# XiaoWang-Github/ORBIT-2

Hardware: AMD Instinct MI355X
Metric: climate-grid samples/sec/node (fwd+bwd), interm_1b ERA5 1.4°→0.25°, 1/2/4/8 GPUs (higher is better)
Workload: dtype bf16

## Files before the change

orbit-2_amd/csrc/common.h:

```cpp
#pragma once
#include <hip/hip_runtime.h>
#include <stdint.h>
#include <type_traits>

#define O2_OK 0
#define O2_ERR_ARG (-1)
#define O2_ERR_LAUNCH (-2)
#define O2_ERR_UNSUPPORTED (-3)

typedef unsigned short bf16_t;
typedef __attribute__((ext_vector_type(8))) short bf16x8;
typedef __attribute__((ext_vector_type(4))) short bf16x4;
typedef __attribute__((ext_vector_type(4))) float f32x4;
typedef __attribute__((ext_vector_type(16))) float f32x16;
typedef __attribute__((ext_vector_type(4))) unsigned int u32x4;
typedef __attribute__((ext_vector_type(2))) unsigned int u32x2;

#define LDS_PTR(T, p) ((__attribute__((address_space(3))) T*)(p))
#define GLB_PTR(T, p) ((const __attribute__((address_space(1))) T*)(p))

__device__ __forceinline__ float bf2f(bf16_t u) { return __uint_as_float(((unsigned)u) << 16); }
__device__ __forceinline__ bf16_t f2bf(float f) { return __builtin_bit_cast(unsigned short, (__bf16)f); }
typedef __attribute__((ext_vector_type(2))) float o2_f32x2;
typedef __attribute__((ext_vector_type(2))) __bf16 o2_bf16x2;
__device__ __forceinline__ unsigned pack_bf2(float lo, float hi) {
  const o2_f32x2 v = {lo, hi};
  return __builtin_bit_cast(unsigned, __builtin_convertvector(v, o2_bf16x2));
}
__device__ __forceinline__ void unpack8(const u32x4 r, float* f) {
#pragma unroll
  for (int k = 0; k < 4; ++k) { f[2 * k] = bf2f((bf16_t)(r[k] & 0xffff)); f[2 * k + 1] = bf2f((bf16_t)(r[k] >> 16)); }
}
__device__ __forceinline__ u32x4 pack8(const float* v) {
  u32x4 o;
#pragma unroll
  for (int k = 0; k < 4; ++k) o[k] = pack_bf2(v[2 * k], v[2 * k + 1]);
  return o;
}

__device__ __forceinline__ void glds16(const void* gsrc, void* lds_wave_base) {
  __builtin_amdgcn_global_load_lds(GLB_PTR(void, gsrc), LDS_PTR(void, lds_wave_base), 16, 0, 0);
}
__device__ __forceinline__ void glds4(const void* gsrc, void* lds_wave_base) {
  __builtin_amdgcn_global_load_lds(GLB_PTR(void, gsrc), LDS_PTR(void, lds_wave_base), 4, 0, 0);
}
__device__ __forceinline__ void glds16_asm(const void* gbase_uniform, uint32_t lane_byte_off, uint32_t lds_dst_uniform) {
  unsigned keep;
  asm volatile("s_mov_b32 %0, m0\n\ts_mov_b32 m0, %3\n\ts_nop 0\n\tglobal_load_lds_dwordx4 %1, %2\n\ts_mov_b32 m0, %0"
               : "=&s"(keep)
               : "v"(lane_byte_off), "s"(gbase_uniform), "s"(lds_dst_uniform)
               : "memory");
}
__device__ __forceinline__ void glds4_asm(const void* gbase_uniform, uint32_t lane_byte_off, uint32_t lds_dst_uniform) {
  unsigned keep;
  asm volatile("s_mov_b32 %0, m0\n\ts_mov_b32 m0, %3\n\ts_nop 0\n\tglobal_load_lds_dword %1, %2\n\ts_mov_b32 m0, %0"
               : "=&s"(keep)
               : "v"(lane_byte_off), "s"(gbase_uniform), "s"(lds_dst_uniform)
               : "memory");
}
__device__ __forceinline__ bf16x4 lds_tr4(const void* lds_addr) {
  return __builtin_amdgcn_ds_read_tr16_b64_v4i16(LDS_PTR(bf16x4, lds_addr));
}

static __device__ uint64_t o2_seed_salt = 0;
#define O2_DEFINE_SALT_OP(tag)                                                                           \
  namespace {                                                                                            \
  __global__ void o2_salt_kernel_##tag(uint64_t v, int add) { o2_seed_salt = add ? o2_seed_salt + v : v; } \
  }                                                                                                      \
  void o2_salt_op_##tag(uint64_t v, int add, hipStream_t s) {                                            \
    hipLaunchKernelGGL(o2_salt_kernel_##tag, dim3(1), dim3(1), 0, s, v, add);                            \
  }
void o2_salt_op_gemm(uint64_t v, int add, hipStream_t s);
void o2_salt_op_attn(uint64_t v, int add, hipStream_t s);
void o2_salt_op_elem(uint64_t v, int add, hipStream_t s);

__device__ __host__ __forceinline__ uint32_t o2_hash(uint32_t seed_lo, uint32_t seed_hi, uint32_t idx_lo,
                                                      uint32_t idx_hi) {
  const uint32_t t = idx_hi ^ seed_hi;
  uint32_t h = idx_lo ^ seed_lo ^ ((t << 16) | (t >> 16)) ^ (t + (t << 3));
  h ^= h >> 16;
  h *= 0x7FEB352Du;
  h ^= h >> 15;
  h *= 0x846CA68Bu;
  h ^= h >> 16;
  return h;
}
__device__ __forceinline__ uint32_t o2_hash64(uint64_t seed, uint64_t idx) {
  return o2_hash((uint32_t)seed, (uint32_t)(seed >> 32), (uint32_t)idx, (uint32_t)(idx >> 32));
}
__device__ __forceinline__ void o2_drop8(float* f, uint64_t salted_seed, int64_t idx, unsigned thr, float dscale) {
  const uint32_t h0 = o2_hash64(salted_seed, (uint64_t)idx >> 2), h1 = o2_hash64(salted_seed, ((uint64_t)idx >> 2) + 1);
#pragma unroll
  for (int j = 0; j < 4; ++j) {
    f[j] = (((h0 >> (8 * j)) & 0xffu) >= thr) ? f[j] * dscale : 0.f;
    f[4 + j] = (((h1 >> (8 * j)) & 0xffu) >= thr) ? f[4 + j] * dscale : 0.f;
  }
}

#define O2_ATTN_KEY_SALT 0x85EBCA6B9E3779B9ull
__device__ __forceinline__ uint32_t o2_attn_rowhash(uint64_t seed, uint64_t row) { return o2_hash64(seed, row); }
__device__ __forceinline__ uint32_t o2_attn_keyhash(uint64_t seed, uint32_t kg) {
  return o2_hash64(seed ^ O2_ATTN_KEY_SALT, (uint64_t)kg);
}
__device__ __forceinline__ uint32_t o2_attn_mix(uint32_t r, uint32_t k) {
  uint32_t x = (r ^ k) * 0x9E3779B1u;
  return x ^ (x >> 16);
}

__device__ __forceinline__ float gelu_f(float x) { return 0.5f * x * (1.0f + erff(x * 0.70710678118654752f)); }
__device__ __forceinline__ float dgelu_f(float x) {
  const float cdf = 0.5f * (1.0f + erff(x * 0.70710678118654752f));
  const float pdf = 0.3989422804014327f * __expf(-0.5f * x * x);
  return cdf + x * pdf;
}

__device__ __forceinline__ float o2_half_erfc_abs(float x, float& e) {
  const float u = fabsf(x) * 0.70710678118654752f;
  const float t = __builtin_amdgcn_rcpf(fmaf(0.3275911f, u, 1.0f));
  float p = fmaf(1.061405429f, t, -1.453152027f);
  p = fmaf(p, t, 1.421413741f);
  p = fmaf(p, t, -0.284496736f);
  p = fmaf(p, t, 0.254829592f);
  e = __builtin_amdgcn_exp2f(x * x * -0.72134752044448170f);
  return 0.5f * p * t * e;
}
__device__ __forceinline__ float gelu_fast(float x) {
  float e;
  const float y = o2_half_erfc_abs(x, e);
  return x * (x > 0.f ? 1.0f - y : y);
}
__device__ __forceinline__ void gelu_both(float x, float& g, float& dg) {
  float e;
  const float y = o2_half_erfc_abs(x, e);
  const float cdf = x > 0.f ? 1.0f - y : y;
  g = x * cdf;
  dg = cdf + x * 0.3989422804014327f * e;
}
__device__ __forceinline__ float dgelu_fast(float x) {
  float e;
  const float y = o2_half_erfc_abs(x, e);
  return (x > 0.f ? 1.0f - y : y) + x * 0.3989422804014327f * e;
}

__device__ __forceinline__ unsigned pack_q14(float lo, float hi) {
  constexpr float MAGIC = 12582912.0f;
  const float a = __builtin_amdgcn_fmed3f(fmaf(lo, 16384.f, MAGIC), MAGIC - 32768.f, MAGIC + 32767.f);
  const float b = __builtin_amdgcn_fmed3f(fmaf(hi, 16384.f, MAGIC), MAGIC - 32768.f, MAGIC + 32767.f);
  return __builtin_amdgcn_perm(__float_as_uint(b), __float_as_uint(a), 0x05040100u);
}
__device__ __forceinline__ void unpack_q14(unsigned w, float& lo, float& hi) {
  lo = (float)(int)(short)(w & 0xffffu) * (1.0f / 16384.f);
  hi = (float)((int)w >> 16) * (1.0f / 16384.f);
}

__device__ __forceinline__ float wave_sum(float v) {
#pragma unroll
  for (int o = 32; o > 0; o >>= 1) v += __shfl_xor(v, o);
  return v;
}
__device__ __forceinline__ float wave_max(float v) {
#pragma unroll
  for (int o = 32; o > 0; o >>= 1) v = fmaxf(v, __shfl_xor(v, o));
  return v;
}
__device__ __forceinline__ float wave_min(float v) {
#pragma unroll
  for (int o = 32; o > 0; o >>= 1) v = fminf(v, __shfl_xor(v, o));
  return v;
}
__device__ __forceinline__ int wave_sum_i(int v) {
#pragma unroll
  for (int o = 32; o > 0; o >>= 1) v += __shfl_xor(v, o);
  return v;
}
__device__ __forceinline__ int64_t wave_sum_i64(int64_t v) {
#pragma unroll
  for (int o = 32; o > 0; o >>= 1) v += (int64_t)__shfl_xor((long long)v, o);
  return v;
}

template <int TPE>
static __global__ __launch_bounds__(256) void o2_sum_parts_kernel(const float* __restrict__ parts, int nparts, int64_t stride,
                                                                  float* __restrict__ out, int64_t nelem, float scale,
                                                                  int accumulate) {
  const int64_t e = ((int64_t)blockIdx.x * 256 + threadIdx.x) / TPE;
  const int j = threadIdx.x % TPE;
  float s = 0.f;
  if (e < nelem)
    for (int k = j; k < nparts; k += TPE) s += parts[(size_t)k * stride + e];
  if (TPE > 1) {
#pragma unroll
    for (int o = TPE / 2; o > 0; o >>= 1) s += __shfl_xor(s, o);
  }
  if (e < nelem && j == 0) out[e] = accumulate ? out[e] + s * scale : s * scale;
}
static inline void o2_sum_parts(const float* parts, int nparts, int64_t stride, float* out, int64_t nelem, float scale,
                                int accumulate, hipStream_t s) {
  if (nparts > 64) {
    hipLaunchKernelGGL(o2_sum_parts_kernel<32>, dim3((unsigned)((nelem * 32 + 255) / 256)), dim3(256), 0, s, parts, nparts,
                       stride, out, nelem, scale, accumulate);
  } else {
    hipLaunchKernelGGL(o2_sum_parts_kernel<1>, dim3((unsigned)((nelem + 255) / 256)), dim3(256), 0, s, parts, nparts, stride,
                       out, nelem, scale, accumulate);
  }
}

template <int V> using o2_int = std::integral_constant<int, V>;
template <class F> static inline void o2_with_flags(F&& f) { f(); }
template <class F, class... Rest> static inline void o2_with_flags(F&& f, bool flag, Rest... rest) {
  if (flag) o2_with_flags([&](auto... c) { f(std::true_type{}, c...); }, rest...);
  else o2_with_flags([&](auto... c) { f(std::false_type{}, c...); }, rest...);
}

static inline int grid_for(int64_t work_items, int per_block, int max_blocks = 4096) {
  int64_t g = (work_items + per_block - 1) / per_block;
  if (g < 1) g = 1;
  if (g > max_blocks) g = max_blocks;
  return (int)g;
}

#define O2_CHECK_LAUNCH()                                   \
  do {                                                      \
    hipError_t e__ = hipGetLastError();                     \
    if (e__ != hipSuccess) return O2_ERR_LAUNCH;            \
  } while (0)
```

orbit-2_amd/csrc/image.hip:

```cpp
#include "score_sums.h"
#include "../../include/orbit2_hip.h"

namespace {

inline int img_grid(int64_t n) { return grid_for(n, 256, 8192); }

template <bool BWD, bool T_FP32 = false>
__global__ __launch_bounds__(256) void unpatchify_kernel(bf16_t* __restrict__ t, float* __restrict__ img, int B, int C,
                                                         int Hh, int Wh, int p) {
  const int64_t per = (int64_t)C * Hh * Wh;
  const int64_t n = (int64_t)B * per;
  const int wf = Wh / p;
  for (int64_t e = (int64_t)blockIdx.x * 256 + threadIdx.x; e < n; e += (int64_t)gridDim.x * 256) {
    const int b = (int)(e / per);
    int64_t r = e - (int64_t)b * per;
    if (!BWD) {
      const int c = (int)(r / ((int64_t)Hh * Wh));
      r -= (int64_t)c * Hh * Wh;
      const int y = (int)(r / Wh), x = (int)(r - (int64_t)y * Wh);
      const int hh = y / p, pp = y - hh * p, ww = x / p, qq = x - ww * p;
      const int64_t ti = ((((int64_t)hh * wf + ww) * p + pp) * p + qq) * C + c;
      img[e] = T_FP32 ? reinterpret_cast<const float*>(t)[(int64_t)b * per + ti] : bf2f(t[(int64_t)b * per + ti]);
    } else {
      const int c = (int)(r % C);
      int64_t q = r / C;
      const int qq = (int)(q % p); q /= p;
      const int pp = (int)(q % p); q /= p;
      const int ww = (int)(q % wf);
      const int hh = (int)(q / wf);
      t[e] = f2bf(img[(int64_t)b * per + ((int64_t)c * Hh + (hh * p + pp)) * Wh + (ww * p + qq)]);
    }
  }
}

constexpr int CONV_MAXCIN = 8;
constexpr int COB = 16;
__global__ __launch_bounds__(256) void conv3x3_fwd_kernel(const float* __restrict__ in, const int* __restrict__ cidx,
                                                          int in_ctotal, const float* __restrict__ wgt,
                                                          const float* __restrict__ bias, float* __restrict__ out,
                                                          float* __restrict__ pre, const float* __restrict__ addend,
                                                          int Ha, int Wa, int B, int Cin, int Cout, int H, int W,
                                                          int mode, int r) {
  __shared__ float sw[COB * CONV_MAXCIN * 9 + COB];
  const int co0 = blockIdx.y * COB;
  const int nco = (Cout - co0) < COB ? (Cout - co0) : COB;
  for (int e = threadIdx.x; e < nco * Cin * 9; e += 256) sw[e] = wgt[(size_t)co0 * Cin * 9 + e];
  for (int e = threadIdx.x; e < nco; e += 256) sw[COB * CONV_MAXCIN * 9 + e] = bias[co0 + e];
  __syncthreads();
  const int64_t npix = (int64_t)B * H * W;
  for (int64_t px = (int64_t)blockIdx.x * 256 + threadIdx.x; px < npix; px += (int64_t)gridDim.x * 256) {
    const int b = (int)(px / ((int64_t)H * W));
    const int rem = (int)(px - (int64_t)b * H * W);
    const int y = rem / W, x = rem - y * W;
    float nb[CONV_MAXCIN][9];
#pragma unroll
    for (int ci = 0; ci < CONV_MAXCIN; ++ci) {
      if (ci < Cin) {
        const int cs = cidx ? cidx[ci] : ci;
        const float* pl = in + ((size_t)b * in_ctotal + cs) * H * W;
#pragma unroll
        for (int k = 0; k < 9; ++k) {
          const int yy = y + k / 3 - 1, xx = x + k % 3 - 1;
          nb[ci][k] = (yy >= 0 && yy < H && xx >= 0 && xx < W) ? pl[(size_t)yy * W + xx] : 0.f;
        }
      }
    }
    for (int co = 0; co < nco; ++co) {
      float acc = sw[COB * CONV_MAXCIN * 9 + co];
#pragma unroll
      for (int ci = 0; ci < CONV_MAXCIN; ++ci) {
        if (ci < Cin) {
#pragma unroll
          for (int k = 0; k < 9; ++k) acc = fmaf(sw[(co * Cin + ci) * 9 + k], nb[ci][k], acc);
        }
      }
      const int cg = co0 + co;
      if (mode == 0) {
        if (addend) acc += addend[(((size_t)b * Cout + cg) * Ha + y) * Wa + x];
        out[(((size_t)b * Cout + cg) * H + y) * W + x] = acc;
      } else {
        pre[(((size_t)b * Cout + cg) * H + y) * W + x] = acc;
        const int rr = r * r;
        const int oc = cg / rr, sub = cg - oc * rr;
        out[(((size_t)b * (Cout / rr) + oc) * (H * r) + (y * r + sub / r)) * (size_t)(W * r) + (x * r + sub % r)] =
            gelu_f(acc);
      }
    }
  }
}

__device__ __forceinline__ float conv_dpre(const float* __restrict__ dout, const float* __restrict__ pre, int b,
                                           int co, int y, int x, int Cout, int H, int W, int mode, int r) {
  if (mode == 0) return dout[(((size_t)b * Cout + co) * H + y) * W + x];
  const int rr = r * r;
  const int oc = co / rr, sub = co - oc * rr;
  const float d =
      dout[(((size_t)b * (Cout / rr) + oc) * (H * r) + (y * r + sub / r)) * (size_t)(W * r) + (x * r + sub % r)];
  return d * dgelu_f(pre[(((size_t)b * Cout + co) * H + y) * W + x]);
}

__global__ __launch_bounds__(256) void conv3x3_bwd_data_kernel(const float* __restrict__ dout,
                                                               const float* __restrict__ pre,
                                                               const float* __restrict__ wgt, float* __restrict__ din,
                                                               int B, int Cin, int Cout, int H, int W, int mode,
                                                               int r) {
  const int64_t n = (int64_t)B * Cin * H * W;
  for (int64_t e = (int64_t)blockIdx.x * 256 + threadIdx.x; e < n; e += (int64_t)gridDim.x * 256) {
    int64_t q = e;
    const int x = (int)(q % W); q /= W;
    const int y = (int)(q % H); q /= H;
    const int ci = (int)(q % Cin);
    const int b = (int)(q / Cin);
    float acc = 0.f;
    for (int co = 0; co < Cout; ++co) {
#pragma unroll
      for (int k = 0; k < 9; ++k) {
        const int yy = y + 1 - k / 3, xx = x + 1 - k % 3;
        if (yy >= 0 && yy < H && xx >= 0 && xx < W)
          acc = fmaf(conv_dpre(dout, pre, b, co, yy, xx, Cout, H, W, mode, r), wgt[((size_t)co * Cin + ci) * 9 + k],
                     acc);
      }
    }
    din[e] = acc;
  }
}

constexpr int TW = 16, TH = 16;
__global__ __launch_bounds__(256) void conv3x3_bwd_weight_kernel(const float* __restrict__ dout,
                                                                 const float* __restrict__ pre,
                                                                 const float* __restrict__ in,
                                                                 const int* __restrict__ cidx, int in_ctotal,
                                                                 float* __restrict__ ws,
                                                                 int B, int Cin, int Cout, int H, int W, int mode,
                                                                 int r) {
  float* dw = ws + ((size_t)blockIdx.y * gridDim.x + blockIdx.x) * ((size_t)Cout * Cin * 9 + Cout);
  float* dbias = dw + (size_t)Cout * Cin * 9;
  __shared__ float sd[COB][TH][TW];
  __shared__ float si[CONV_MAXCIN][TH + 2][TW + 2];
  const int tiles_x = (W + TW - 1) / TW;
  const int ty0 = (blockIdx.x / tiles_x) * TH, tx0 = (blockIdx.x % tiles_x) * TW;
  const int b = blockIdx.y;
  for (int e = threadIdx.x; e < Cin * (TH + 2) * (TW + 2); e += 256) {
    const int ci = e / ((TH + 2) * (TW + 2));
    const int rem = e - ci * (TH + 2) * (TW + 2);
    const int yy = ty0 + rem / (TW + 2) - 1, xx = tx0 + rem % (TW + 2) - 1;
    const int cs = cidx ? cidx[ci] : ci;
    si[ci][rem / (TW + 2)][rem % (TW + 2)] =
        (yy >= 0 && yy < H && xx >= 0 && xx < W) ? in[(((size_t)b * in_ctotal + cs) * H + yy) * W + xx] : 0.f;
  }
  for (int co0 = 0; co0 < Cout; co0 += COB) {
    const int nco = (Cout - co0) < COB ? (Cout - co0) : COB;
    __syncthreads();
    for (int e = threadIdx.x; e < nco * TH * TW; e += 256) {
      const int co = e / (TH * TW);
      const int rem = e - co * TH * TW;
      const int y = ty0 + rem / TW, x = tx0 + rem % TW;
      sd[co][rem / TW][rem % TW] =
          (y < H && x < W) ? conv_dpre(dout, pre, b, co0 + co, y, x, Cout, H, W, mode, r) : 0.f;
    }
    __syncthreads();
    for (int e = threadIdx.x; e < nco * Cin * 9; e += 256) {
      const int co = e / (Cin * 9);
      const int rem = e - co * Cin * 9;
      const int ci = rem / 9, k = rem - ci * 9;
      const int ky = k / 3, kx = k - ky * 3;
      float s = 0.f;
      for (int y = 0; y < TH; ++y)
#pragma unroll
        for (int x = 0; x < TW; ++x) s = fmaf(sd[co][y][x], si[ci][y + ky][x + kx], s);
      dw[((size_t)(co0 + co) * Cin + ci) * 9 + k] = s;
    }
    for (int co = threadIdx.x; co < nco; co += 256) {
      float s = 0.f;
      for (int y = 0; y < TH; ++y)
        for (int x = 0; x < TW; ++x) s += sd[co][y][x];
      dbias[co0 + co] = s;
    }
  }
}

__global__ __launch_bounds__(256) void clamp_channel_kernel(float* __restrict__ img, const float* __restrict__ ref,
                                                            float* __restrict__ dimg, int B, int C, int HW,
                                                            int chan) {
  const int64_t n = (int64_t)B * HW;
  for (int64_t e = (int64_t)blockIdx.x * 256 + threadIdx.x; e < n; e += (int64_t)gridDim.x * 256) {
    const int b = (int)(e / HW);
    const size_t off = ((size_t)b * C + chan) * HW + (e - (int64_t)b * HW);
    if (dimg) { if (!(ref[off] > 0.f)) dimg[off] = 0.f; }
    else img[off] = fmaxf(img[off], 0.f);
  }
}


__global__ __launch_bounds__(256) void loss_fwd_kernel(const float* __restrict__ pred, const float* __restrict__ tgt,
                                                       int Ht, int Wt, const float* __restrict__ latw,
                                                       const float* __restrict__ chanw, float* __restrict__ part,
                                                       float* __restrict__ part2, int C, int H, int W, int kind) {
  const int plane = blockIdx.y;
  const int c = plane % C, b = plane / C;
  const float* p = pred + (size_t)plane * H * W;
  const float* t = tgt + ((size_t)b * C + c) * Ht * Wt;
  const float cw = chanw ? chanw[c] : 1.f;
  float s = 0.f, s2 = 0.f;
  for (int e = blockIdx.x * 256 + threadIdx.x; e < H * W; e += gridDim.x * 256) {
    const int i = e / W, j = e - i * W;
    const float pv = p[e];
    const float tv0 = t[(size_t)i * Wt + j];
    const float d = pv - tv0;
    float err = d * d;
    if (kind == 2) {
      if (j < W - 1) s2 += fabsf((t[(size_t)i * Wt + j + 1] - tv0) - (p[e + 1] - pv));
      if (i < H - 1) s2 += fabsf((t[(size_t)(i + 1) * Wt + j] - tv0) - (p[e + W] - pv));
    }
    if (kind == 1) {
      float tv = 0.f;
      if (i < H - 1) {
        tv += fabsf(p[e + W] - pv);
        if (j < W - 1) tv += 0.7f * fabsf(p[e + W + 1] - pv);
        if (j >= 1) tv += 0.7f * fabsf(p[e + W - 1] - pv);
      }
      if (j < W - 1) tv += fabsf(p[e + 1] - pv);
      err += 0.02f * tv;
    }
    s += err * (latw ? latw[i] : 1.f) * cw;
  }
  s = wave_sum(s);
  s2 = wave_sum(s2);
  __shared__ float sw[8];
  if ((threadIdx.x & 63) == 0) { sw[threadIdx.x >> 6] = s; sw[4 + (threadIdx.x >> 6)] = s2; }
  __syncthreads();
  if (threadIdx.x == 0) {
    part[(size_t)plane * gridDim.x + blockIdx.x] = sw[0] + sw[1] + sw[2] + sw[3];
    part2[(size_t)plane * gridDim.x + blockIdx.x] = sw[4] + sw[5] + sw[6] + sw[7];
  }
}

__global__ void loss_final_kernel(const float* __restrict__ part, const float* __restrict__ part2, int nblk, int B,
                                  int C, int HW, const float* __restrict__ chanw, int kind, float* __restrict__ out) {
  float tot = 0.f;
  for (int c = 0; c < C; ++c) {
    float s = 0.f;
    for (int e = threadIdx.x; e < B * nblk; e += 64) {
      const int b = e / nblk, k = e - b * nblk;
      s += part[((size_t)(b * C + c)) * nblk + k];
    }
    s = wave_sum(s);
    if (threadIdx.x == 0) out[c] = s / ((float)B * (float)HW);
    tot += s;
  }
  float agg = tot / ((float)B * (float)C * (float)HW);
  if (kind == 2) {
    float s2 = 0.f;
    for (int e = threadIdx.x; e < B * C * nblk; e += 64) s2 += part2[e];
    s2 = wave_sum(s2);
    float cwm = 1.f;
    if (chanw) { cwm = 0.f; for (int c = 0; c < C; ++c) cwm += chanw[c]; cwm /= (float)C; }
    agg += 0.1f * (s2 / ((float)B * (float)C * (float)HW)) * cwm;
  }
  if (threadIdx.x == 0) out[C] = agg;
}

__global__ __launch_bounds__(256) void loss_bwd_kernel(const float* __restrict__ pred, const float* __restrict__ tgt,
                                                       int Ht, int Wt, const float* __restrict__ latw,
                                                       const float* __restrict__ chanw,
                                                       const float* __restrict__ gscale, float* __restrict__ dpred,
                                                       int B, int C, int H, int W, int kind) {
  const int64_t n = (int64_t)B * C * H * W;
  const float g0 = gscale[0] / (float)n;
  for (int64_t e = (int64_t)blockIdx.x * 256 + threadIdx.x; e < n; e += (int64_t)gridDim.x * 256) {
    int64_t q = e;
    const int j = (int)(q % W); q /= W;
    const int i = (int)(q % H); q /= H;
    const int c = (int)(q % C);
    const int b = (int)(q / C);
    const float* p = pred + ((size_t)b * C + c) * H * W;
    const int o = i * W + j;
    const float pv = p[o];
    const float wi = latw ? latw[i] : 1.f;
    const float wim = (latw && i > 0) ? latw[i - 1] : 1.f;
    float g = 2.f * (pv - tgt[(((size_t)b * C + c) * Ht + i) * Wt + j]) * wi;
    if (kind == 2) {
      const float* t = tgt + ((size_t)b * C + c) * Ht * Wt;
      const float tv0 = t[(size_t)i * Wt + j];
      float gs = 0.f;
      if (j < W - 1) gs += sgn((t[(size_t)i * Wt + j + 1] - tv0) - (p[o + 1] - pv));
      if (j > 0) gs -= sgn((tv0 - t[(size_t)i * Wt + j - 1]) - (pv - p[o - 1]));
      if (i < H - 1) gs += sgn((t[(size_t)(i + 1) * Wt + j] - tv0) - (p[o + W] - pv));
      if (i > 0) gs -= sgn((tv0 - t[(size_t)(i - 1) * Wt + j]) - (pv - p[o - W]));
      float cwm = 1.f;
      if (chanw) { cwm = 0.f; for (int cc = 0; cc < C; ++cc) cwm += chanw[cc]; cwm /= (float)C; }
      dpred[e] = (g * (chanw ? chanw[c] : 1.f) + 0.1f * cwm * gs) * g0;
      continue;
    }
    if (kind == 1) {
      float tv = 0.f;
      if (i < H - 1) {
        tv -= sgn(p[o + W] - pv) * wi;
        if (j < W - 1) tv -= 0.7f * sgn(p[o + W + 1] - pv) * wi;
        if (j >= 1) tv -= 0.7f * sgn(p[o + W - 1] - pv) * wi;
      }
      if (j < W - 1) tv -= sgn(p[o + 1] - pv) * wi;
      if (j > 0) tv += sgn(pv - p[o - 1]) * wi;
      if (i > 0) {
        tv += sgn(pv - p[o - W]) * wim;
        if (j > 0) tv += 0.7f * sgn(pv - p[o - W - 1]) * wim;
        if (j < W - 1) tv += 0.7f * sgn(pv - p[o - W + 1]) * wim;
      }
      g += 0.02f * tv;
    }
    dpred[e] = g * (chanw ? chanw[c] : 1.f) * g0;
  }
}

}

extern "C" int orbit2_unpatchify_fwd(const void* t, float* img, int B, int C, int h, int w, int p, int s,
                                     void* stream) {
  if (!t || !img || B <= 0 || C <= 0 || p <= 0 || s <= 0 || (h * s) % p || (w * s) % p) return O2_ERR_ARG;
  const int64_t n = (int64_t)B * C * h * s * w * s;
  hipLaunchKernelGGL(unpatchify_kernel<false>, dim3(img_grid(n)), dim3(256), 0, (hipStream_t)stream, (bf16_t*)t,
                     img, B, C, h * s, w * s, p);
  O2_CHECK_LAUNCH();
  return O2_OK;
}
extern "C" int orbit2_unpatchify_fwd_f32(const float* t, float* img, int B, int C, int h, int w, int p, int s,
                                         void* stream) {
  if (!t || !img || B <= 0 || C <= 0 || p <= 0 || s <= 0 || (h * s) % p || (w * s) % p) return O2_ERR_ARG;
  const int64_t n = (int64_t)B * C * h * s * w * s;
  hipLaunchKernelGGL((unpatchify_kernel<false, true>), dim3(img_grid(n)), dim3(256), 0, (hipStream_t)stream,
                     (bf16_t*)t, img, B, C, h * s, w * s, p);
  O2_CHECK_LAUNCH();
  return O2_OK;
}
extern "C" int orbit2_unpatchify_bwd(const float* dimg, void* dt, int B, int C, int h, int w, int p, int s,
                                     void* stream) {
  if (!dimg || !dt || B <= 0 || C <= 0 || p <= 0 || s <= 0 || (h * s) % p || (w * s) % p) return O2_ERR_ARG;
  const int64_t n = (int64_t)B * C * h * s * w * s;
  hipLaunchKernelGGL(unpatchify_kernel<true>, dim3(img_grid(n)), dim3(256), 0, (hipStream_t)stream, (bf16_t*)dt,
                     (float*)dimg, B, C, h * s, w * s, p);
  O2_CHECK_LAUNCH();
  return O2_OK;
}

extern "C" int orbit2_conv3x3_fwd(const float* in, const int* chan_idx, int in_ctotal, const float* weight,
                                  const float* bias, float* out, float* pre, const float* addend, int Ha, int Wa,
                                  int B, int Cin, int Cout, int H, int W, int mode, int r, void* stream) {
  if (!in || !weight || !bias || !out || B <= 0 || Cin <= 0 || Cin > CONV_MAXCIN || Cout <= 0 || H <= 0 || W <= 0)
    return O2_ERR_ARG;
  if (mode == 1 && (!pre || r <= 0 || Cout % (r * r))) return O2_ERR_ARG;
  if (mode != 0 && mode != 1) return O2_ERR_ARG;
  if (addend && (mode != 0 || Ha < H || Wa < W)) return O2_ERR_ARG;
  dim3 grid(img_grid((int64_t)B * H * W), (Cout + COB - 1) / COB);
  hipLaunchKernelGGL(conv3x3_fwd_kernel, grid, dim3(256), 0, (hipStream_t)stream, in, chan_idx, in_ctotal, weight,
                     bias, out, pre, addend, Ha, Wa, B, Cin, Cout, H, W, mode, r);
  O2_CHECK_LAUNCH();
  return O2_OK;
}

extern "C" int64_t orbit2_conv3x3_bwd_ws_floats(int B, int Cin, int Cout, int H, int W) {
  if (B <= 0 || Cin <= 0 || Cout <= 0 || H <= 0 || W <= 0) return 0;
  return (int64_t)B * ((W + TW - 1) / TW) * ((H + TH - 1) / TH) * ((int64_t)Cout * Cin * 9 + Cout);
}

extern "C" int orbit2_conv3x3_bwd(const float* dout, const float* in, const int* chan_idx, int in_ctotal,
                                  const float* weight, const float* pre, float* din, float* dweight, float* dbias,
                                  int B, int Cin, int Cout, int H, int W, int mode, int r, float* ws, void* stream) {
  if (!dout || !in || !weight || !dweight || !dbias || !ws || B <= 0 || Cin <= 0 || Cin > CONV_MAXCIN || Cout <= 0)
    return O2_ERR_ARG;
  if (mode == 1 && (!pre || r <= 0 || Cout % (r * r))) return O2_ERR_ARG;
  if (mode != 0 && mode != 1) return O2_ERR_ARG;
  hipStream_t s = (hipStream_t)stream;
  if (din) {
    hipLaunchKernelGGL(conv3x3_bwd_data_kernel, dim3(img_grid((int64_t)B * Cin * H * W)), dim3(256), 0, s, dout,
                       pre, weight, din, B, Cin, Cout, H, W, mode, r);
    O2_CHECK_LAUNCH();
  }
  dim3 grid(((W + TW - 1) / TW) * ((H + TH - 1) / TH), B);
  hipLaunchKernelGGL(conv3x3_bwd_weight_kernel, grid, dim3(256), 0, s, dout, pre, in, chan_idx, in_ctotal, ws,
                     B, Cin, Cout, H, W, mode, r);
  const int nparts = (int)(grid.x * grid.y);
  const int64_t nw = (int64_t)Cout * Cin * 9, slab = nw + Cout;
  o2_sum_parts(ws, nparts, slab, dweight, nw, 1.0f, 1, s);
  o2_sum_parts(ws + nw, nparts, slab, dbias, Cout, 1.0f, 1, s);
  O2_CHECK_LAUNCH();
  return O2_OK;
}

extern "C" int orbit2_clamp_channel(float* img, int B, int C, int HW, int chan, void* stream) {
  if (!img || B <= 0 || C <= 0 || HW <= 0 || chan < 0 || chan >= C) return O2_ERR_ARG;
  hipLaunchKernelGGL(clamp_channel_kernel, dim3(img_grid((int64_t)B * HW)), dim3(256), 0, (hipStream_t)stream,
                     img, (const float*)nullptr, (float*)nullptr, B, C, HW, chan);
  O2_CHECK_LAUNCH();
  return O2_OK;
}
extern "C" int orbit2_clamp_channel_bwd(const float* img_clamped, float* dimg, int B, int C, int HW, int chan,
                                        void* stream) {
  if (!img_clamped || !dimg || B <= 0 || C <= 0 || HW <= 0 || chan < 0 || chan >= C) return O2_ERR_ARG;
  hipLaunchKernelGGL(clamp_channel_kernel, dim3(img_grid((int64_t)B * HW)), dim3(256), 0, (hipStream_t)stream,
                     (float*)nullptr, img_clamped, dimg, B, C, HW, chan);
  O2_CHECK_LAUNCH();
  return O2_OK;
}

extern "C" int orbit2_loss_fwd(const float* pred, const float* target, int Ht, int Wt, const float* lat_w,
                               const float* chan_w, float* out, float* ws, int B, int C, int H, int W, int kind,
                               void* stream) {
  if (!o2_pair_ok(pred, target, B, C, H, W, Ht, Wt) || !out || !ws) return O2_ERR_ARG;
  if (kind < 0 || kind > 2) return O2_ERR_ARG;
  hipStream_t s = (hipStream_t)stream;
  float* ws2 = ws + (size_t)B * C * ORBIT2_LOSS_BLOCKS;
  hipLaunchKernelGGL(loss_fwd_kernel, dim3(ORBIT2_LOSS_BLOCKS, B * C), dim3(256), 0, s, pred, target, Ht, Wt, lat_w, chan_w, ws,
                     ws2, C, H, W, kind);
  O2_CHECK_LAUNCH();
  hipLaunchKernelGGL(loss_final_kernel, dim3(1), dim3(64), 0, s, ws, ws2, ORBIT2_LOSS_BLOCKS, B, C, H * W, chan_w, kind, out);
  O2_CHECK_LAUNCH();
  return O2_OK;
}

extern "C" int orbit2_loss_bwd(const float* pred, const float* target, int Ht, int Wt, const float* lat_w,
                               const float* chan_w, const float* gscale, float* dpred, int B, int C, int H, int W,
                               int kind, void* stream) {
  if (!o2_pair_ok(pred, target, B, C, H, W, Ht, Wt) || !gscale || !dpred) return O2_ERR_ARG;
  if (kind < 0 || kind > 2) return O2_ERR_ARG;
  hipLaunchKernelGGL(loss_bwd_kernel, dim3(img_grid((int64_t)B * C * H * W)), dim3(256), 0, (hipStream_t)stream,
                     pred, target, Ht, Wt, lat_w, chan_w, gscale, dpred, B, C, H, W, kind);
  O2_CHECK_LAUNCH();
  return O2_OK;
}

namespace {
constexpr int EVAL_NM = O2_NMOMENTS;
__global__ __launch_bounds__(256) void eval_moments_kernel(const float* __restrict__ pred, const float* __restrict__ target,
                                                           int Ht, int Wt, const float* __restrict__ lat_w,
                                                           const float* __restrict__ clim, double* __restrict__ out,
                                                           int C, int H, int W) {
  const int bc = blockIdx.y;
  const float* p = pred + (size_t)bc * H * W;
  const float* t = target + (size_t)bc * Ht * Wt;
  const float* cl = clim ? clim + (size_t)(bc % C) * H * W : nullptr;
  float s[EVAL_NM];
#pragma unroll
  for (int k = 0; k < EVAL_NM; ++k) s[k] = 0.f;
  for (int i = blockIdx.x * 256 + threadIdx.x; i < H * W; i += gridDim.x * 256) {
    const int y = i / W, x = i - y * W;
    const float c0 = cl ? cl[i] : 0.f;
    o2_moments_add(s, p[i] - c0, t[(size_t)y * Wt + x] - c0, lat_w ? lat_w[y] : 1.f);
  }
  o2_block_sums_add(s, out + (size_t)bc * EVAL_NM);
}
}

extern "C" int orbit2_eval_moments(const float* pred, const float* target, int Ht, int Wt, const float* lat_w,
                                   const float* clim, double* out, int B, int C, int H, int W, void* stream) {
  if (!o2_pair_ok(pred, target, B, C, H, W, Ht, Wt) || !out) return O2_ERR_ARG;
  hipStream_t s = (hipStream_t)stream;
  if (hipMemsetAsync(out, 0, sizeof(double) * (size_t)B * C * EVAL_NM, s) != hipSuccess) return O2_ERR_LAUNCH;
  hipLaunchKernelGGL(eval_moments_kernel, dim3(o2_image_blocks((int64_t)H * W), B * C), dim3(256), 0, s, pred, target, Ht, Wt,
                     lat_w, clim, out, C, H, W);
  O2_CHECK_LAUNCH();
  return O2_OK;
}

namespace {
__device__ __forceinline__ void welford_step(float x, float& mean, float& m2, float kf) {
  const float d = x - mean;
  mean += d / kf;
  m2 = fmaf(d, x - mean, m2);
}

__global__ __launch_bounds__(256) void ensemble_update_kernel(const float* __restrict__ member, float* __restrict__ mean,
                                                              float* __restrict__ m2, int64_t n, int64_t n4, int k) {
  const float kf = (float)k;
  const int64_t tid = (int64_t)blockIdx.x * 256 + threadIdx.x, nthr = (int64_t)gridDim.x * 256;
  const f32x4* x4 = reinterpret_cast<const f32x4*>(member);
  f32x4* mean4 = reinterpret_cast<f32x4*>(mean);
  f32x4* m24 = reinterpret_cast<f32x4*>(m2);
  if (k == 1) {
    const f32x4 zero = {0.f, 0.f, 0.f, 0.f};
    for (int64_t i = tid; i < n4; i += nthr) {
      mean4[i] = x4[i];
      m24[i] = zero;
    }
    for (int64_t i = 4 * n4 + tid; i < n; i += nthr) {
      mean[i] = member[i];
      m2[i] = 0.f;
    }
    return;
  }
  for (int64_t i = tid; i < n4; i += nthr) {
    const f32x4 x = x4[i];
    f32x4 mu = mean4[i], s = m24[i];
#pragma unroll
    for (int j = 0; j < 4; ++j) {
      float mj = mu[j], sj = s[j];
      welford_step(x[j], mj, sj, kf);
      mu[j] = mj;
      s[j] = sj;
    }
    mean4[i] = mu;
    m24[i] = s;
  }
  for (int64_t i = 4 * n4 + tid; i < n; i += nthr) {
    float mu = mean[i], s = m2[i];
    welford_step(member[i], mu, s, kf);
    mean[i] = mu;
    m2[i] = s;
  }
}
}

extern "C" int orbit2_ensemble_update(const float* member, float* mean, float* m2, int64_t n, int k, void* stream) {
  if (!member || !mean || !m2 || n <= 0 || k < 1 || member == mean || member == m2 || mean == m2) return O2_ERR_ARG;
  const bool aligned = (((uintptr_t)member | (uintptr_t)mean | (uintptr_t)m2) & 15) == 0;
  const int64_t n4 = aligned ? n / 4 : 0;
  const int64_t lanes = n4 > 0 ? n4 : n;
  int64_t nblk = (lanes + 255) / 256;
  if (nblk > 2048) nblk = 2048;
  hipLaunchKernelGGL(ensemble_update_kernel, dim3((unsigned)nblk), dim3(256), 0, (hipStream_t)stream, member, mean, m2, n, n4,
                     k);
  O2_CHECK_LAUNCH();
  return O2_OK;
}

namespace {
constexpr int GS_NM = 4;
__global__ __launch_bounds__(256) void gaussian_scores_kernel(const float* __restrict__ mean, const float* __restrict__ std_,
                                                              const float* __restrict__ target, int Ht, int Wt,
                                                              const float* __restrict__ lat_w, double* __restrict__ out, int H,
                                                              int W) {
  const int bc = blockIdx.y;
  const float* m = mean + (size_t)bc * H * W;
  const float* sd = std_ + (size_t)bc * H * W;
  const float* t = target + (size_t)bc * Ht * Wt;
  float s[GS_NM] = {0.f, 0.f, 0.f, 0.f};
  for (int i = blockIdx.x * 256 + threadIdx.x; i < H * W; i += gridDim.x * 256) {
    const int y = i / W, x = i - y * W;
    const float sg = sd[i];
    const float d = t[(size_t)y * Wt + x] - m[i];
    const float w = lat_w ? lat_w[y] : 1.f;
    const float ad = fabsf(d);
    float crps = ad;
    if (sg > 0.f) {
      const float z = ad / sg;
      const float phi = 0.3989422804014327f * expf(-0.5f * z * z);
      crps = ad * erff(z * 0.70710678118654752f) + sg * (2.f * phi - 0.5641895835477563f);
    }
    s[0] += w * crps;
    s[1] += w * sg * sg;
    s[2] += w * d * d;
    s[3] += ad <= sg ? 1.f : 0.f;
  }
  o2_block_sums_add(s, out + (size_t)bc * GS_NM);
}
}

extern "C" int orbit2_gaussian_scores(const float* mean, const float* std_, const float* target, int Ht, int Wt,
                                      const float* lat_w, double* out, int B, int C, int H, int W, void* stream) {
  if (!o2_pair_ok(mean, target, B, C, H, W, Ht, Wt) || !std_ || !out) return O2_ERR_ARG;
  if ((int64_t)B * C > 65535 || (int64_t)H * W > (int64_t)INT32_MAX - 64 * 256) return O2_ERR_ARG;
  hipStream_t s = (hipStream_t)stream;
  if (hipMemsetAsync(out, 0, sizeof(double) * (size_t)B * C * GS_NM, s) != hipSuccess) return O2_ERR_LAUNCH;
  hipLaunchKernelGGL(gaussian_scores_kernel, dim3(o2_image_blocks((int64_t)H * W), B * C), dim3(256), 0, s, mean, std_, target, Ht,
                     Wt, lat_w, out, H, W);
  O2_CHECK_LAUNCH();
  return O2_OK;
}

namespace {
constexpr int PE_MAX_SIDE = 2048;

__device__ __forceinline__ void cubic_taps(int o, int n_in, int n_out, int idx[4], float w[4]) {
  const float scale = (float)n_in / (float)n_out;
  const float s = scale * ((float)o + 0.5f) - 0.5f;
  const float fl = floorf(s);
  const float t = s - fl;
  const int base = (int)fl;
  constexpr float A = -0.75f;
  const float x0 = t + 1.0f, x1 = t, x2 = 1.0f - t, x3 = 2.0f - t;
  w[0] = ((A * x0 - 5.0f * A) * x0 + 8.0f * A) * x0 - 4.0f * A;
  w[1] = ((A + 2.0f) * x1 - (A + 3.0f)) * x1 * x1 + 1.0f;
  w[2] = ((A + 2.0f) * x2 - (A + 3.0f)) * x2 * x2 + 1.0f;
  w[3] = ((A * x3 - 5.0f * A) * x3 + 8.0f * A) * x3 - 4.0f * A;
#pragma unroll
  for (int k = 0; k < 4; ++k) {
    int i = base - 1 + k;
    idx[k] = i < 0 ? 0 : (i > n_in - 1 ? n_in - 1 : i);
  }
}

template <bool SAME>
__global__ __launch_bounds__(256) void posembed_fwd_kernel(const float* __restrict__ pe, const float* __restrict__ sw,
                                                           const float* __restrict__ sb, float res, float* __restrict__ out,
                                                           int oh, int ow, int nh, int nw, int D) {
  const int pix = blockIdx.x, oy = pix / nw, ox = pix - oy * nw;
  int iy[4], ix[4];
  float wy[4], wx[4];
  if (!SAME) {
    cubic_taps(oy, oh, nh, iy, wy);
    cubic_taps(ox, ow, nw, ix, wx);
  }
  float* o = out + (size_t)pix * D;
  for (int d = threadIdx.x * 4; d < D; d += 256 * 4) {
    float4 acc;
    if (SAME) {
      acc = *reinterpret_cast<const float4*>(pe + (size_t)pix * D + d);
    } else {
      acc = make_float4(0.f, 0.f, 0.f, 0.f);
#pragma unroll
      for (int a = 0; a < 4; ++a) {
        const float* row = pe + ((size_t)iy[a] * ow) * D + d;
        float4 r = make_float4(0.f, 0.f, 0.f, 0.f);
#pragma unroll
        for (int b = 0; b < 4; ++b) {
          const float4 v = *reinterpret_cast<const float4*>(row + (size_t)ix[b] * D);
          r.x += v.x * wx[b]; r.y += v.y * wx[b]; r.z += v.z * wx[b]; r.w += v.w * wx[b];
        }
        acc.x += r.x * wy[a]; acc.y += r.y * wy[a]; acc.z += r.z * wy[a]; acc.w += r.w * wy[a];
      }
    }
    if (sw) {
      const float4 w4 = *reinterpret_cast<const float4*>(sw + d), b4 = *reinterpret_cast<const float4*>(sb + d);
      acc.x += w4.x * res + b4.x; acc.y += w4.y * res + b4.y; acc.z += w4.z * res + b4.z; acc.w += w4.w * res + b4.w;
    }
    *reinterpret_cast<float4*>(o + d) = acc;
  }
}

__global__ __launch_bounds__(256) void posembed_bwd_kernel(const float* __restrict__ dout, float* __restrict__ dpe, int oh, int ow,
                                                           int nh, int nw, int D) {
  __shared__ float wyd[PE_MAX_SIDE], wxd[PE_MAX_SIDE];
  const int pix = blockIdx.x, sy = pix / ow, sx = pix - sy * ow;
  for (int o = threadIdx.x; o < nh; o += 256) {
    int idx[4];
    float w[4], s = 0.f;
    cubic_taps(o, oh, nh, idx, w);
#pragma unroll
    for (int k = 0; k < 4; ++k) s += (idx[k] == sy) ? w[k] : 0.f;
    wyd[o] = s;
  }
  for (int o = threadIdx.x; o < nw; o += 256) {
    int idx[4];
    float w[4], s = 0.f;
    cubic_taps(o, ow, nw, idx, w);
#pragma unroll
    for (int k = 0; k < 4; ++k) s += (idx[k] == sx) ? w[k] : 0.f;
    wxd[o] = s;
  }
  __syncthreads();
  for (int d = threadIdx.x * 4; d < D; d += 256 * 4) {
    float4 acc = make_float4(0.f, 0.f, 0.f, 0.f);
    for (int oy = 0; oy < nh; ++oy) {
      const float wy = wyd[oy];
      if (wy == 0.f) continue;
      float4 r = make_float4(0.f, 0.f, 0.f, 0.f);
      for (int ox = 0; ox < nw; ++ox) {
        const float wx = wxd[ox];
        if (wx == 0.f) continue;
        const float4 v = *reinterpret_cast<const float4*>(dout + ((size_t)oy * nw + ox) * D + d);
        r.x += v.x * wx; r.y += v.y * wx; r.z += v.z * wx; r.w += v.w * wx;
      }
      acc.x += r.x * wy; acc.y += r.y * wy; acc.z += r.z * wy; acc.w += r.w * wy;
    }
    *reinterpret_cast<float4*>(dpe + (size_t)pix * D + d) = acc;
  }
}
}

extern "C" int orbit2_posembed_fwd(const float* pe, const float* sw, const float* sb, float res, float* out, int oh, int ow,
                                   int nh, int nw, int D, void* stream) {
  if (!pe || !out || (sw == nullptr) != (sb == nullptr) || oh <= 0 || ow <= 0 || nh <= 0 || nw <= 0 || D <= 0 || (D & 3))
    return O2_ERR_ARG;
  if (nh > PE_MAX_SIDE || nw > PE_MAX_SIDE || oh > PE_MAX_SIDE || ow > PE_MAX_SIDE) return O2_ERR_UNSUPPORTED;
  hipStream_t s = (hipStream_t)stream;
  if (oh == nh) {
    if (ow != nw) return O2_ERR_ARG;
    hipLaunchKernelGGL((posembed_fwd_kernel<true>), dim3(nh * nw), dim3(256), 0, s, pe, sw, sb, res, out, oh, ow, nh, nw, D);
  } else {
    hipLaunchKernelGGL((posembed_fwd_kernel<false>), dim3(nh * nw), dim3(256), 0, s, pe, sw, sb, res, out, oh, ow, nh, nw, D);
  }
  O2_CHECK_LAUNCH();
  return O2_OK;
}

extern "C" int orbit2_posembed_bwd(const float* dout, float* dpe, int oh, int ow, int nh, int nw, int D, void* stream) {
  if (!dout || !dpe || oh <= 0 || ow <= 0 || nh <= 0 || nw <= 0 || D <= 0 || (D & 3)) return O2_ERR_ARG;
  if (nh > PE_MAX_SIDE || nw > PE_MAX_SIDE || oh > PE_MAX_SIDE || ow > PE_MAX_SIDE) return O2_ERR_UNSUPPORTED;
  hipStream_t s = (hipStream_t)stream;
  if (oh == nh) {
    if (ow != nw) return O2_ERR_ARG;
    if (hipMemcpyAsync(dpe, dout, sizeof(float) * (size_t)nh * nw * D, hipMemcpyDeviceToDevice, s) != hipSuccess) return O2_ERR_LAUNCH;
    return O2_OK;
  }
  hipLaunchKernelGGL(posembed_bwd_kernel, dim3(oh * ow), dim3(256), 0, s, dout, dpe, oh, ow, nh, nw, D);
  O2_CHECK_LAUNCH();
  return O2_OK;
}
```

Measured before the change: 17.72.

## Tile 3x3 conv kernels through LDS and restructure weight-grad partial reduction

The forward conv now stages an input tile plus halo in shared memory instead of reading nine neighbours per pixel from global memory, and weights are read straight from global. The data-gradient kernel switches from one thread per (ci,pixel), which looped over all output channels with repeated global reads, to a tiled kernel that stages dpre tiles in LDS and accumulates every input channel per pixel. It uses a wave-uniform fast path that skips bounds checks away from the image border. The weight-gradient kernel packs several spatial tiles per block to raise thread utilisation and writes partials element-major, so a new contiguous reduction kernel sums them. This adds register pressure and dynamic shared memory, and forward weight reads now go through cache rather than LDS.

```diff
diff --git a/orbit-2_amd/csrc/common.h b/orbit-2_amd/csrc/common.h
--- a/orbit-2_amd/csrc/common.h
+++ b/orbit-2_amd/csrc/common.h
@@ -179,15 +179,22 @@
   return v;
 }
 
-template <int TPE>
-static __global__ __launch_bounds__(256) void o2_sum_parts_kernel(const float* __restrict__ parts, int nparts, int64_t stride,
-                                                                  float* __restrict__ out, int64_t nelem, float scale,
-                                                                  int accumulate) {
-  const int64_t e = ((int64_t)blockIdx.x * 256 + threadIdx.x) / TPE;
+template <int TPE, bool EM = false, int NT = 256>
+static __global__ __launch_bounds__(NT) void o2_sum_parts_kernel(const float* __restrict__ parts, int nparts, int64_t stride,
+                                                                 float* __restrict__ out, int64_t nelem, float scale,
+                                                                 int accumulate) {
+  const int64_t e = ((int64_t)blockIdx.x * NT + threadIdx.x) / TPE;
   const int j = threadIdx.x % TPE;
   float s = 0.f;
-  if (e < nelem)
-    for (int k = j; k < nparts; k += TPE) s += parts[(size_t)k * stride + e];
+  if (e < nelem) {
+    if (EM) {
+      const float* p = parts + (size_t)e * nparts;
+#pragma unroll 8
+      for (int k = j; k < nparts; k += TPE) s += p[k];
+    } else {
+      for (int k = j; k < nparts; k += TPE) s += parts[(size_t)k * stride + e];
+    }
+  }
   if (TPE > 1) {
 #pragma unroll
     for (int o = TPE / 2; o > 0; o >>= 1) s += __shfl_xor(s, o);
@@ -204,6 +211,16 @@
                        out, nelem, scale, accumulate);
   }
 }
+static inline void o2_sum_parts_em(const float* parts, int nparts, float* out, int64_t nelem, float scale, int accumulate,
+                                   hipStream_t s) {
+  if (nparts > 64) {
+    hipLaunchKernelGGL((o2_sum_parts_kernel<32, true, 64>), dim3((unsigned)((nelem * 32 + 63) / 64)), dim3(64), 0, s, parts,
+                       nparts, (int64_t)0, out, nelem, scale, accumulate);
+  } else {
+    hipLaunchKernelGGL((o2_sum_parts_kernel<1, true, 64>), dim3((unsigned)((nelem + 63) / 64)), dim3(64), 0, s, parts, nparts,
+                       (int64_t)0, out, nelem, scale, accumulate);
+  }
+}
 
 template <int V> using o2_int = std::integral_constant<int, V>;
 template <class F> static inline void o2_with_flags(F&& f) { f(); }
diff --git a/orbit-2_amd/csrc/image.hip b/orbit-2_amd/csrc/image.hip
--- a/orbit-2_amd/csrc/image.hip
+++ b/orbit-2_amd/csrc/image.hip
@@ -35,46 +35,60 @@
 
 constexpr int CONV_MAXCIN = 8;
 constexpr int COB = 16;
+constexpr int CT_W = 64, CT_H = 8;
+constexpr int CT_LW = CT_W + 2, CT_LH = CT_H + 2;
+constexpr int CT_ROWS = CT_H / 4;
+
+inline dim3 conv_tile_grid(int B, int H, int W, int ny) {
+  return dim3((unsigned)((int64_t)B * ((W + CT_W - 1) / CT_W) * ((H + CT_H - 1) / CT_H)), (unsigned)ny);
+}
+
 __global__ __launch_bounds__(256) void conv3x3_fwd_kernel(const float* __restrict__ in, const int* __restrict__ cidx,
                                                           int in_ctotal, const float* __restrict__ wgt,
                                                           const float* __restrict__ bias, float* __restrict__ out,
                                                           float* __restrict__ pre, const float* __restrict__ addend,
                                                           int Ha, int Wa, int B, int Cin, int Cout, int H, int W,
                                                           int mode, int r) {
-  __shared__ float sw[COB * CONV_MAXCIN * 9 + COB];
+  __shared__ float si[CONV_MAXCIN][CT_LH][CT_LW];
+  const int tiles_x = (W + CT_W - 1) / CT_W, tiles = tiles_x * ((H + CT_H - 1) / CT_H);
+  const int b = blockIdx.x / tiles, t = blockIdx.x - b * tiles;
+  const int ty0 = (t / tiles_x) * CT_H, tx0 = (t % tiles_x) * CT_W;
   const int co0 = blockIdx.y * COB;
   const int nco = (Cout - co0) < COB ? (Cout - co0) : COB;
-  for (int e = threadIdx.x; e < nco * Cin * 9; e += 256) sw[e] = wgt[(size_t)co0 * Cin * 9 + e];
-  for (int e = threadIdx.x; e < nco; e += 256) sw[COB * CONV_MAXCIN * 9 + e] = bias[co0 + e];
+  for (int e = threadIdx.x; e < Cin * CT_LH * CT_LW; e += 256) {
+    const int ci = e / (CT_LH * CT_LW);
+    const int rem = e - ci * (CT_LH * CT_LW);
+    const int ly = rem / CT_LW, lx = rem - ly * CT_LW;
+    const int yy = ty0 + ly - 1, xx = tx0 + lx - 1;
+    const int cs = cidx ? cidx[ci] : ci;
+    si[ci][ly][lx] =
+        (yy >= 0 && yy < H && xx >= 0 && xx < W) ? in[(((size_t)b * in_ctotal + cs) * H + yy) * W + xx] : 0.f;
+  }
   __syncthreads();
-  const int64_t npix = (int64_t)B * H * W;
-  for (int64_t px = (int64_t)blockIdx.x * 256 + threadIdx.x; px < npix; px += (int64_t)gridDim.x * 256) {
-    const int b = (int)(px / ((int64_t)H * W));
-    const int rem = (int)(px - (int64_t)b * H * W);
-    const int y = rem / W, x = rem - y * W;
+  const int lx = threadIdx.x & 63, x = tx0 + lx;
+#pragma unroll 1
+  for (int ly = threadIdx.x >> 6; ly < CT_H; ly += 4) {
+    const int y = ty0 + ly;
+    if (y >= H || x >= W) continue;
     float nb[CONV_MAXCIN][9];
 #pragma unroll
     for (int ci = 0; ci < CONV_MAXCIN; ++ci) {
       if (ci < Cin) {
-        const int cs = cidx ? cidx[ci] : ci;
-        const float* pl = in + ((size_t)b * in_ctotal + cs) * H * W;
-#pragma unroll
-        for (int k = 0; k < 9; ++k) {
-          const int yy = y + k / 3 - 1, xx = x + k % 3 - 1;
-          nb[ci][k] = (yy >= 0 && yy < H && xx >= 0 && xx < W) ? pl[(size_t)yy * W + xx] : 0.f;
-        }
+#pragma unroll
+        for (int k = 0; k < 9; ++k) nb[ci][k] = si[ci][ly + k / 3][lx + k % 3];
       }
     }
     for (int co = 0; co < nco; ++co) {
-      float acc = sw[COB * CONV_MAXCIN * 9 + co];
+      const int cg = co0 + co;
+      const float* wc = wgt + (size_t)cg * Cin * 9;
+      float acc = bias[cg];
 #pragma unroll
       for (int ci = 0; ci < CONV_MAXCIN; ++ci) {
         if (ci < Cin) {
 #pragma unroll
-          for (int k = 0; k < 9; ++k) acc = fmaf(sw[(co * Cin + ci) * 9 + k], nb[ci][k], acc);
+          for (int k = 0; k < 9; ++k) acc = fmaf(wc[ci * 9 + k], nb[ci][k], acc);
         }
       }
-      const int cg = co0 + co;
       if (mode == 0) {
         if (addend) acc += addend[(((size_t)b * Cout + cg) * Ha + y) * Wa + x];
         out[(((size_t)b * Cout + cg) * H + y) * W + x] = acc;
@@ -99,82 +113,147 @@
   return d * dgelu_f(pre[(((size_t)b * Cout + co) * H + y) * W + x]);
 }
 
+template <bool CHECK>
+__device__ __forceinline__ void conv_din_taps(const float (*sd)[CT_LH][CT_LW], const float* __restrict__ wgt, int co0, int nco,
+                                              int Cin, int ly, int lx, int y, int x, int H, int W,
+                                              float (&acc)[CONV_MAXCIN]) {
+  for (int co = 0; co < nco; ++co) {
+    const float* wc = wgt + (size_t)(co0 + co) * Cin * 9;
+    float d[9];
+#pragma unroll
+    for (int k = 0; k < 9; ++k) d[k] = sd[co][ly + 2 - k / 3][lx + 2 - k % 3];
+#pragma unroll
+    for (int ci = 0; ci < CONV_MAXCIN; ++ci) {
+      if (ci < Cin) {
+#pragma unroll
+        for (int k = 0; k < 9; ++k) {
+          const int yy = y + 1 - k / 3, xx = x + 1 - k % 3;
+          if (!CHECK || (yy >= 0 && yy < H && xx >= 0 && xx < W)) acc[ci] = fmaf(d[k], wc[ci * 9 + k], acc[ci]);
+        }
+      }
+    }
+  }
+}
+
 __global__ __launch_bounds__(256) void conv3x3_bwd_data_kernel(const float* __restrict__ dout,
                                                                const float* __restrict__ pre,
                                                                const float* __restrict__ wgt, float* __restrict__ din,
                                                                int B, int Cin, int Cout, int H, int W, int mode,
                                                                int r) {
-  const int64_t n = (int64_t)B * Cin * H * W;
-  for (int64_t e = (int64_t)blockIdx.x * 256 + threadIdx.x; e < n; e += (int64_t)gridDim.x * 256) {
-    int64_t q = e;
-    const int x = (int)(q % W); q /= W;
-    const int y = (int)(q % H); q /= H;
-    const int ci = (int)(q % Cin);
-    const int b = (int)(q / Cin);
-    float acc = 0.f;
-    for (int co = 0; co < Cout; ++co) {
-#pragma unroll
-      for (int k = 0; k < 9; ++k) {
-        const int yy = y + 1 - k / 3, xx = x + 1 - k % 3;
-        if (yy >= 0 && yy < H && xx >= 0 && xx < W)
-          acc = fmaf(conv_dpre(dout, pre, b, co, yy, xx, Cout, H, W, mode, r), wgt[((size_t)co * Cin + ci) * 9 + k],
-                     acc);
-      }
-    }
-    din[e] = acc;
+  __shared__ float sd[COB][CT_LH][CT_LW];
+  const int tiles_x = (W + CT_W - 1) / CT_W, tiles = tiles_x * ((H + CT_H - 1) / CT_H);
+  const int b = blockIdx.x / tiles, t = blockIdx.x - b * tiles;
+  const int ty0 = (t / tiles_x) * CT_H, tx0 = (t % tiles_x) * CT_W;
+  const int lx = threadIdx.x & 63, x = tx0 + lx;
+  const int wy = threadIdx.x >> 6;
+  float acc[CT_ROWS][CONV_MAXCIN];
+#pragma unroll
+  for (int j = 0; j < CT_ROWS; ++j)
+#pragma unroll
+    for (int ci = 0; ci < CONV_MAXCIN; ++ci) acc[j][ci] = 0.f;
+  for (int co0 = 0; co0 < Cout; co0 += COB) {
+    const int nco = (Cout - co0) < COB ? (Cout - co0) : COB;
+    __syncthreads();
+    for (int e = threadIdx.x; e < nco * CT_LH * CT_LW; e += 256) {
+      const int co = e / (CT_LH * CT_LW);
+      const int rem = e - co * (CT_LH * CT_LW);
+      const int ly = rem / CT_LW, llx = rem - ly * CT_LW;
+      const int yy = ty0 + ly - 1, xx = tx0 + llx - 1;
+      sd[co][ly][llx] =
+          (yy >= 0 && yy < H && xx >= 0 && xx < W) ? conv_dpre(dout, pre, b, co0 + co, yy, xx, Cout, H, W, mode, r) : 0.f;
+    }
+    __syncthreads();
+#pragma unroll
+    for (int j = 0; j < CT_ROWS; ++j) {
+      const int ly = wy + 4 * j, y = ty0 + ly;
+      if (y < H && x < W) {
+        const bool border = y == 0 || y == H - 1 || x == 0 || x == W - 1;
+        if (__ballot(border) == 0) conv_din_taps<false>(sd, wgt, co0, nco, Cin, ly, lx, y, x, H, W, acc[j]);
+        else conv_din_taps<true>(sd, wgt, co0, nco, Cin, ly, lx, y, x, H, W, acc[j]);
+      }
+    }
+  }
+#pragma unroll
+  for (int j = 0; j < CT_ROWS; ++j) {
+    const int y = ty0 + wy + 4 * j;
+    if (y < H && x < W) {
+#pragma unroll
+      for (int ci = 0; ci < CONV_MAXCIN; ++ci)
+        if (ci < Cin) din[(((size_t)b * Cin + ci) * H + y) * W + x] = acc[j][ci];
+    }
   }
 }
 
 constexpr int TW = 16, TH = 16;
+constexpr int TI = (TH + 2) * (TW + 2);
+constexpr int WG_MAXTILES = 4;
+
+inline int conv_wgrad_group(int Cin, int Cout) {
+  const int g = 256 / ((Cout < COB ? Cout : COB) * Cin * 9);
+  return g < 1 ? 1 : (g > WG_MAXTILES ? WG_MAXTILES : g);
+}
+
 __global__ __launch_bounds__(256) void conv3x3_bwd_weight_kernel(const float* __restrict__ dout,
                                                                  const float* __restrict__ pre,
                                                                  const float* __restrict__ in,
                                                                  const int* __restrict__ cidx, int in_ctotal,
                                                                  float* __restrict__ ws,
                                                                  int B, int Cin, int Cout, int H, int W, int mode,
-                                                                 int r) {
-  float* dw = ws + ((size_t)blockIdx.y * gridDim.x + blockIdx.x) * ((size_t)Cout * Cin * 9 + Cout);
-  float* dbias = dw + (size_t)Cout * Cin * 9;
-  __shared__ float sd[COB][TH][TW];
-  __shared__ float si[CONV_MAXCIN][TH + 2][TW + 2];
+                                                                 int r, int G) {
+  extern __shared__ __attribute__((aligned(16))) float wsm[];
+  const int ncb = Cout < COB ? Cout : COB;
+  float* sd = wsm;
+  float* si = wsm + (size_t)G * ncb * TH * TW;
   const int tiles_x = (W + TW - 1) / TW;
-  const int ty0 = (blockIdx.x / tiles_x) * TH, tx0 = (blockIdx.x % tiles_x) * TW;
-  const int b = blockIdx.y;
-  for (int e = threadIdx.x; e < Cin * (TH + 2) * (TW + 2); e += 256) {
-    const int ci = e / ((TH + 2) * (TW + 2));
-    const int rem = e - ci * (TH + 2) * (TW + 2);
-    const int yy = ty0 + rem / (TW + 2) - 1, xx = tx0 + rem % (TW + 2) - 1;
+  const int tiles = tiles_x * ((H + TH - 1) / TH);
+  const int nparts = B * tiles;
+  const int part0 = blockIdx.x * G;
+  const int ng = (nparts - part0) < G ? (nparts - part0) : G;
+  const size_t nw = (size_t)Cout * Cin * 9;
+  for (int e = threadIdx.x; e < ng * Cin * TI; e += 256) {
+    const int g = e / (Cin * TI);
+    const int q = e - g * Cin * TI;
+    const int ci = q / TI, rem = q - ci * TI;
+    const int b = (part0 + g) / tiles, t = (part0 + g) - b * tiles;
+    const int yy = (t / tiles_x) * TH + rem / (TW + 2) - 1, xx = (t % tiles_x) * TW + rem % (TW + 2) - 1;
     const int cs = cidx ? cidx[ci] : ci;
-    si[ci][rem / (TW + 2)][rem % (TW + 2)] =
-        (yy >= 0 && yy < H && xx >= 0 && xx < W) ? in[(((size_t)b * in_ctotal + cs) * H + yy) * W + xx] : 0.f;
+    si[e] = (yy >= 0 && yy < H && xx >= 0 && xx < W) ? in[(((size_t)b * in_ctotal + cs) * H + yy) * W + xx] : 0.f;
   }
   for (int co0 = 0; co0 < Cout; co0 += COB) {
     const int nco = (Cout - co0) < COB ? (Cout - co0) : COB;
     __syncthreads();
-    for (int e = threadIdx.x; e < nco * TH * TW; e += 256) {
-      const int co = e / (TH * TW);
-      const int rem = e - co * TH * TW;
-      const int y = ty0 + rem / TW, x = tx0 + rem % TW;
-      sd[co][rem / TW][rem % TW] =
+    for (int e = threadIdx.x; e < ng * nco * TH * TW; e += 256) {
+      const int g = e / (nco * TH * TW);
+      const int q = e - g * nco * TH * TW;
+      const int co = q / (TH * TW), rem = q - co * TH * TW;
+      const int b = (part0 + g) / tiles, t = (part0 + g) - b * tiles;
+      const int y = (t / tiles_x) * TH + rem / TW, x = (t % tiles_x) * TW + rem % TW;
+      sd[(g * ncb + co) * TH * TW + rem] =
           (y < H && x < W) ? conv_dpre(dout, pre, b, co0 + co, y, x, Cout, H, W, mode, r) : 0.f;
     }
     __syncthreads();
-    for (int e = threadIdx.x; e < nco * Cin * 9; e += 256) {
-      const int co = e / (Cin * 9);
-      const int rem = e - co * Cin * 9;
+    const int ne = nco * Cin * 9;
+    for (int e = threadIdx.x; e < ng * ne; e += 256) {
+      const int g = e / ne;
+      const int q = e - g * ne;
+      const int co = q / (Cin * 9);
+      const int rem = q - co * Cin * 9;
       const int ci = rem / 9, k = rem - ci * 9;
       const int ky = k / 3, kx = k - ky * 3;
+      const float* d = sd + (g * ncb + co) * TH * TW;
+      const float* a = si + (g * Cin + ci) * TI + ky * (TW + 2) + kx;
       float s = 0.f;
       for (int y = 0; y < TH; ++y)
 #pragma unroll
-        for (int x = 0; x < TW; ++x) s = fmaf(sd[co][y][x], si[ci][y + ky][x + kx], s);
-      dw[((size_t)(co0 + co) * Cin + ci) * 9 + k] = s;
-    }
-    for (int co = threadIdx.x; co < nco; co += 256) {
+        for (int x = 0; x < TW; ++x) s = fmaf(d[y * TW + x], a[y * (TW + 2) + x], s);
+      ws[(((size_t)(co0 + co) * Cin + ci) * 9 + k) * nparts + part0 + g] = s;
+    }
+    for (int e = 255 - threadIdx.x; e < ng * nco; e += 256) {
+      const int g = e / nco, co = e - g * nco;
+      const float* d = sd + (g * ncb + co) * TH * TW;
       float s = 0.f;
-      for (int y = 0; y < TH; ++y)
-        for (int x = 0; x < TW; ++x) s += sd[co][y][x];
-      dbias[co0 + co] = s;
+      for (int i = 0; i < TH * TW; ++i) s += d[i];
+      ws[(nw + co0 + co) * nparts + part0 + g] = s;
     }
   }
 }
@@ -350,9 +429,9 @@
   if (mode == 1 && (!pre || r <= 0 || Cout % (r * r))) return O2_ERR_ARG;
   if (mode != 0 && mode != 1) return O2_ERR_ARG;
   if (addend && (mode != 0 || Ha < H || Wa < W)) return O2_ERR_ARG;
-  dim3 grid(img_grid((int64_t)B * H * W), (Cout + COB - 1) / COB);
-  hipLaunchKernelGGL(conv3x3_fwd_kernel, grid, dim3(256), 0, (hipStream_t)stream, in, chan_idx, in_ctotal, weight,
-                     bias, out, pre, addend, Ha, Wa, B, Cin, Cout, H, W, mode, r);
+  hipLaunchKernelGGL(conv3x3_fwd_kernel, conv_tile_grid(B, H, W, (Cout + COB - 1) / COB), dim3(256), 0,
+                     (hipStream_t)stream, in, chan_idx, in_ctotal, weight, bias, out, pre, addend, Ha, Wa, B, Cin, Cout,
+                     H, W, mode, r);
   O2_CHECK_LAUNCH();
   return O2_OK;
 }
@@ -371,17 +450,21 @@
   if (mode != 0 && mode != 1) return O2_ERR_ARG;
   hipStream_t s = (hipStream_t)stream;
   if (din) {
-    hipLaunchKernelGGL(conv3x3_bwd_data_kernel, dim3(img_grid((int64_t)B * Cin * H * W)), dim3(256), 0, s, dout,
-                       pre, weight, din, B, Cin, Cout, H, W, mode, r);
+    hipLaunchKernelGGL(conv3x3_bwd_data_kernel, conv_tile_grid(B, H, W, 1), dim3(256), 0, s, dout, pre, weight, din,
+                       B, Cin, Cout, H, W, mode, r);
     O2_CHECK_LAUNCH();
   }
-  dim3 grid(((W + TW - 1) / TW) * ((H + TH - 1) / TH), B);
-  hipLaunchKernelGGL(conv3x3_bwd_weight_kernel, grid, dim3(256), 0, s, dout, pre, in, chan_idx, in_ctotal, ws,
-                     B, Cin, Cout, H, W, mode, r);
-  const int nparts = (int)(grid.x * grid.y);
-  const int64_t nw = (int64_t)Cout * Cin * 9, slab = nw + Cout;
-  o2_sum_parts(ws, nparts, slab, dweight, nw, 1.0f, 1, s);
-  o2_sum_parts(ws + nw, nparts, slab, dbias, Cout, 1.0f, 1, s);
+  const int64_t nparts64 = (int64_t)B * ((W + TW - 1) / TW) * ((H + TH - 1) / TH);
+  if (nparts64 > INT32_MAX) return O2_ERR_ARG;
+  const int nparts = (int)nparts64;
+  const int G = conv_wgrad_group(Cin, Cout);
+  const size_t shm = sizeof(float) * (size_t)G * ((size_t)(Cout < COB ? Cout : COB) * TH * TW + (size_t)Cin * TI);
+  hipLaunchKernelGGL(conv3x3_bwd_weight_kernel, dim3((unsigned)((nparts + G - 1) / G)), dim3(256), shm, s, dout, pre,
+                     in, chan_idx, in_ctotal, ws, B, Cin, Cout, H, W, mode, r, G);
+  O2_CHECK_LAUNCH();
+  const int64_t nw = (int64_t)Cout * Cin * 9;
+  o2_sum_parts_em(ws, nparts, dweight, nw, 1.0f, 1, s);
+  o2_sum_parts_em(ws + nw * nparts, nparts, dbias, Cout, 1.0f, 1, s);
   O2_CHECK_LAUNCH();
   return O2_OK;
 }
```

New measurement: 17.79, median of 6. No clear change (+0.4%).
